# GestaltCogTeam/STEP

Hardware: AMD Instinct MI355X
Metric: training windows/sec on PEMS04, horizon-12 MAE parity, 1/2/4/8 MI355X (higher is better)
Workload: dtype f16 (TSFormer Q/K/weights) + bf16 (P, V, GraphWaveNet / graph-learner GEMMs) operands, f32 accumulate

## Files before the change

### include/step_hip.h

```cpp
#ifndef STEP_HIP_H
#define STEP_HIP_H

#include <stdint.h>

#ifdef __cplusplus
extern "C" {
#endif

const char* step_last_error(void);
int step_abi_version(void);

typedef struct StepGemm {
    int M, N, K, batch;
    const void* A; long sam, sak, sab; int a_bf16;
    const void* B; long sbk, sbn, sbb; int b_bf16;
    float* C; long ldc, scn, scb;
    float alpha;
    int accumulate;
    const float* bias; int relu;
    int splitk;
    int a_kblk; long a_kstride;
    int b_kblk; long b_kstride;
    int b_nblk; long b_nstride;
    int c_nblk; long c_nstride;
// ... 37 lines not shown
    float *bn3_w, *bn3_b, *bn3_rm, *bn3_rv;
    float *fc_out_w, *fc_out_b;
    float *fc_cat_w, *fc_cat_b;
    int gemm_bf16;
} StepDglParams;

long step_dgl_global_saved_floats(int N, int T);
long step_dgl_global_work_floats(int N, int T, int backward);
int step_dgl_global_forward(const float* series_nt, int N, int T, const StepDglParams* p, int training,
                            float momentum, float* saved, float* work, float* g, void* stream);
int step_dgl_global_backward(const float* series_nt, int N, int T, const StepDglParams* p, const float* saved,
                             const float* dg, float* work, const StepDglParams* grads, void* stream);
#define STEP_DGL_FRESH_FC_GRAD 16
int step_dgl_global_backward_phase(const float* series_nt, int N, int T, const StepDglParams* p, const float* saved,
                             const float* dg, float* work, const StepDglParams* grads, int phase, void* stream);

typedef struct StepDglShard { int own1; double count1, count2; } StepDglShard;
int step_dgl_global_forward_shard(const float* series_slice, int N, int Ts, const StepDglParams* p, int training, float momentum,
                                  float* saved, float* work, double* sums, float* g, const StepDglShard* shard, int phase,
                                  void* stream);
int step_dgl_global_backward_shard(const float* series_slice, int N, int Ts, const StepDglParams* p, const float* saved,
                                   const float* dg, float* work, const StepDglParams* grads, const StepDglShard* shard, int phase,
                                   void* stream);
long step_dgl_global_offset(int N, int T, int item);

long step_dgl_edges_saved_floats(int B, int N);
long step_dgl_edges_work_floats(int N);
long step_dgl_edges_theta_offset(int N);
int step_dgl_edges_forward(const float* g, int N, int B, const StepDglParams* p, const float* u, uint64_t seed,
                           float temperature, float* saved, float* theta_out, float* adj_out, void* stream);
int step_dgl_edges_backward(const float* g, int N, int B, const StepDglParams* p, const float* saved,
                            const float* dtheta, const float* dadj, float temperature, float* work,
                            const StepDglParams* grads, float* dg, void* aux_stream, void* stream);
int step_dgl_edges_backward_acc(const float* g, int N, int B, const StepDglParams* p, const float* saved,
                                const float* dtheta, const float* dadj, float temperature, float* work,
                                const StepDglParams* grads, float* dg, int dg_accumulate, void* aux_stream, void* stream);

typedef struct StepGwnetParams {
    float *nodevec1, *nodevec2;
    float *start_w, *start_b;
    float *filter_w[8], *filter_b[8];
    float *gate_w[8], *gate_b[8];
    float *skip_w[8], *skip_b[8];
    float *bn_w[8], *bn_b[8], *bn_rm[8], *bn_rv[8];
    float *gconv_w[8], *gconv_b[8];
    float *fc_his0_w, *fc_his0_b, *fc_his2_w, *fc_his2_b;
    float *end1_w, *end1_b, *end2_w, *end2_b;
    int gemm_bf16;
} StepGwnetParams;

long step_gwnet_saved_floats(int B, int N, int dropout);
long step_gwnet_work_floats(int B, int N, int backward);
long step_gwnet_saved_offset(int B, int N, int dropout, int item, int layer);
int step_gwnet_forward(const float* hist, int B, int N, int Cin, const float* hidden_last, const float* adj,
                       const StepGwnetParams* p, int training, float dropout_p, uint64_t seed, float momentum,
                       float* saved, float* work, float* pred, void* stream);
int step_gwnet_forward_phase(const float* hist, int B, int N, int Cin, const float* hidden_last, const float* adj,
                             const StepGwnetParams* p, int training, float dropout_p, uint64_t seed, float momentum,
                             float* saved, float* work, float* pred, int phase, void* stream);
int step_gwnet_backward(const float* hist, int B, int N, int Cin, const float* hidden_last, const StepGwnetParams* p,
                        const float* saved, float* work, const float* dpred, const StepGwnetParams* grads,
                        float* dadj, int dropout, void* aux_stream, void* leaf_stream, void* stream);

int step_pt_dropout(const float* x, float* y, long n, float p, uint64_t seed, uint32_t site, void* stream);
int step_pt_ffn_hidden_fwd(const float* x, const float* w1, const float* b1, long R, float p, uint64_t seed, uint32_t site,
                           uint16_t* hidden, void* stream);
int step_pt_ffn_hidden_bwd(const float* dy, const float* w2, const uint16_t* hidden, long R, float p, uint16_t* dhidden, void* stream);
int step_pt_colsum_bf16(const uint16_t* x, long rows, int cols, float* out, void* stream);
long step_pt_rows_linear_pack_bytes(int nkc, int nog);
int step_pt_rows_linear_pack(const float* w, long swo, long swi, int nkc, int nog, const float* bias, void* pack, void* stream);
int step_pt_rows_linear(const void* x, int x_bf16, long R, const void* pack, int nkc, int nog, void* y, int y_bf16, int accumulate, void* stream);
int step_pt_layer_pack(const float* wi, const float* bi, const float* wo, const float* bo, const float* w1, const float* b1, const float* w2,
                       const float* b2, void* ffn, void* qkv, void* o, void* da, void* dx, void* stream);
long step_pt_proj_wgrad_ws_floats(long R);
int step_pt_proj_wgrad(const float* x, const uint16_t* dqkv, const float* dov, const uint16_t* a, long R, float* ws, float* dwi, float* dbi, float* dwo,
                       void* stream);
int step_pt_ffn_fused_fwd_ln(const float* h1, long R, const void* pack, float p, const uint64_t* pool, long pool_words, uint64_t seed, uint32_t site_hidden,
                             uint32_t site_out, const float* gamma, const float* beta, float* pre, float* y, float* stats, void* stream);
int step_pt_rows_linear_ln(const uint16_t* x, long R, const void* pack, const float* res, float p, uint64_t seed, uint32_t site, const float* gamma,
                           const float* beta, float* pre, float* y, float* stats, void* stream);
int step_pt_embed_unmasked_fwd(const float* series, const int* um, const float* w, const float* b, const float* pos, long S, int L, int Pu, float p,
                               uint64_t seed, uint32_t site, float* x, void* stream);
int step_pt_embed_unmasked_bwd(const float* dx, const float* series, const int* um, long S, int L, int Pu, float p, uint64_t seed, uint32_t site,
                               float* dpos, float* dw, float* db, void* stream);
int step_pt_dec_input_bwd_sums(const float* dout, long S, int P, int Pu, float p, uint64_t seed, uint32_t site, const int* midx, float* dz, float* dpos,
                               float* dmask, void* stream);
long step_pt_ffn_pack_bytes(void);
long step_pt_ffn_wgrad_workgroups(long R);
long step_pt_ffn_wgrad_ws_floats(long R);
int step_pt_ffn_pack(const float* w1, const float* b1, const float* w2, const float* b2, void* pack, void* stream);
int step_pt_ffn_fused_fwd(const float* h1, long R, const void* pack, float p, const uint64_t* pool, long pool_words, uint64_t seed, uint32_t site,
                          float* f2, void* stream);
int step_pt_ffn_fused_bwd_data(const float* df2, const float* h1, long R, const void* pack, float p, const uint64_t* pool, long pool_words,
                               uint64_t seed, uint32_t site, float* dh1, void* stream);
int step_pt_ffn_fused_bwd_weights(const float* df2, const float* h1, long R, const void* pack, const float* b1, float p, const uint64_t* pool,
                                  long pool_words, uint64_t seed, uint32_t site, float* ws, float* dw1, float* db1, float* dw2, void* stream);
int step_pt_dropout_relu_mask(float* d, const float* relu_of, long n, float p, uint64_t seed, uint32_t site, void* stream);
int step_pt_add_dropout(const float* a, const float* b, float* out, long n, float p, uint64_t seed, uint32_t site, void* stream);
int step_pt_add_rows(float* x, long S, int P, const float* vec, const int* idx, void* stream);
int step_pt_sum_over_seq(const float* dx, long S, int ldp, int p_off, int p_cnt, const int* idx, float* dvec, void* stream);
int step_pt_token_gather(const float* src, long S, int P, const int* idx, int T, float scale, float* dst, void* stream);
int step_pt_token_scatter(const float* ddst, long S, int P, const int* idx, int T, float scale, float* dsrc, void* stream);
int step_pt_dec_input(const float* z, const float* mask_token, const float* pos, const int* midx, long S, int P, int Pu,
                      float p, uint64_t seed, uint32_t site, float* out, void* stream);
int step_pt_dec_input_bwd(const float* dout, long S, int P, int Pu, float p, uint64_t seed, uint32_t site, float* dz,
                          float* dm, void* stream);
// ... 103 lines not shown
```

### step_amd/csrc/gwnet.hip

```cpp
#include "common.h"
#include "step_internal.h"
#include <vector>

namespace {

constexpr int C = 32, CAT = 224, CS = 256, CE = 512, OUT = 12, NL = 8, HID = 96;
constexpr int TIN[NL] = {13, 12, 10, 9, 7, 6, 4, 3};
constexpr int DIL[NL] = {1, 2, 1, 2, 1, 2, 1, 2};
constexpr int TOUT[NL] = {12, 10, 9, 7, 6, 4, 3, 1};

__global__ void start_conv_kernel(const float* __restrict__ hist, int B, int N, int Cin, const float* __restrict__ w,
                                  const float* __restrict__ b, float* __restrict__ x0) {
    long idx = (long)blockIdx.x * 256 + threadIdx.x;
    long total = (long)B * N * 13 * C;
    if (idx >= total) return;
    int c = idx % C, t = (idx / C) % 13;
    long bn = idx / (C * 13);
    int n = bn % N, bb = bn / N;
    float v = b[c];
    if (t >= 1) {
        const float* src = hist + (((long)bb * 12 + (t - 1)) * N + n) * Cin;
        v += w[c * 2] * src[0] + w[c * 2 + 1] * src[1];
    }
    x0[idx] = v;
// ... 542 lines not shown
        long o[4];
        bool valid[4];
#pragma unroll
        for (int u = 0; u < 4; ++u) {
            const int j = j0 + 8 * u + jg;
            const int g = j / Tin, t = j - g * Tin;
            const long bnr = bn0 + g;
            valid[u] = j < njt && bnr < BN;
            const long bc = valid[u] ? bnr : 0;
            const int tc = valid[u] ? t : 0;
            o[u] = (bc * Tin + tc) * C + c;
            const bool tap1 = valid[u] && tc >= dil;
            dr[u] = (dres && tap1) ? dres[(bc * Tout + tc - dil) * C + c] : 0.f;
            yv[u] = yprev ? yprev[o[u]] : 0.f;
            float x = 0.f;
            if (valid[u] && tc < Tout) x += dxs[g * Tout + tc][c];
            if (tap1) x += dxs[g * Tout + tc - dil][32 + c];
            v[u] = x;
        }
#pragma unroll
        for (int u = 0; u < 4; ++u) {
            if (!valid[u]) continue;
            const float x = v[u] + dr[u];
            dx[o[u]] = x;
            s1 += x; s2 += x * (yv[u] - mean) * rstd;
        }
    }
    if (!yprev) return;
    red[jg][c] = s1; red[jg][32 + c] = s2;
    __syncthreads();
    if (threadIdx.x < 64) {
        float a = 0.f;
#pragma unroll
        for (int r = 0; r < 8; ++r) a += red[r][threadIdx.x];
        bsum[threadIdx.x] = a;
    }
    __syncthreads();
    add_block_sums(sums, bsum);
}

__global__ void im2col_kernel(XIn x, long BN, int Tin, int Tout, int dil, float* __restrict__ xcat) {
    long idx = (long)blockIdx.x * 256 + threadIdx.x;
    if (idx >= BN * Tout * 64) return;
    int k = idx % 64, t = (idx / 64) % Tout;
    long bn = idx / (64L * Tout);
    float v = x.src[(bn * Tin + t + (k >> 5) * dil) * C + (k & 31)];
    if (x.stat) v = v * x.stat[k & 31] + x.stat[32 + (k & 31)];
    xcat[idx] = v;
}
__global__ void unpack_skip_grad_kernel(const float* __restrict__ dwskip, SkipPtrs G) {
    const int o = blockIdx.x, k = threadIdx.x;
    G.w[k >> 5][o * C + (k & 31)] += dwskip[o * CS + k];
}
__global__ void head_combine_kernel(const float* __restrict__ skip, const float* __restrict__ h2, long n, float* __restrict__ xh) {
    long idx = (long)blockIdx.x * 256 + threadIdx.x;
    if (idx >= n) return;
    xh[idx] = fmaxf(skip[idx] + h2[idx], 0.f);
}
struct MPtr8 { float* p[8]; };
__global__ void add_to8_kernel(MPtr8 dst, const float* __restrict__ v, int n) {
    int i = blockIdx.x * 256 + threadIdx.x;
    if (i >= n) return;
    const float x = v[i];
#pragma unroll
    for (int k = 0; k < 8; ++k) dst.p[k][i] += x;
}
__global__ void relu_bwd_kernel(float* __restrict__ d, const float* __restrict__ y, long n) {
    long idx = (long)blockIdx.x * 256 + threadIdx.x;
    if (idx < n && !(y[idx] > 0.f)) d[idx] = 0.f;
}

__global__ __launch_bounds__(256) void rowsum_mod_kernel(const float* __restrict__ x, int cols, int mod, float* __restrict__ out) {
    __shared__ float red[4];
    const long row = blockIdx.x;
    float s = 0.f;
    for (int j = threadIdx.x; j < cols; j += 256) s += x[row * cols + j];
    s = wave_sum(s);
    if ((threadIdx.x & 63) == 0) red[threadIdx.x >> 6] = s;
    __syncthreads();
    if (threadIdx.x == 0) atomicAdd(&out[row % mod], red[0] + red[1] + red[2] + red[3]);
}

constexpr int ADJ_NSEG = 2 * (12 + 10 + 9 + 7 + 6 + 4 + 3);
struct AdjOffsets { long cat[NL - 1], dcat[NL - 1]; };
__global__ void adj_ktab_kernel(AdjOffsets o, int N, GemmKSeg* __restrict__ tab) {
    const int j = threadIdx.x, s = blockIdx.x;
    if (j >= ADJ_NSEG) return;
    constexpr int tout[NL - 1] = {12, 10, 9, 7, 6, 4, 3};
    int i = 0, rem = j >> 1;
    while (rem >= tout[i]) { rem -= tout[i]; ++i; }
    const int t = rem, pair = j & 1, T = tout[i];
    GemmKSeg g;
    g.a_off = o.cat[i] + (long)t * CAT + (pair == 0 ? (1 + 2 * s) * C : 0);
    g.b_off = o.dcat[i] + (long)t * CAT + (pair == 0 ? (2 + 2 * s) * C : (1 + 2 * s) * C);
    g.a_rs = g.b_rs = T * CAT;
    g.a_bs = g.b_bs = (long)N * T * CAT;
    tab[s * ADJ_NSEG + j] = g;
}

inline dim3 g1(long n) { return dim3((unsigned)((n + 255) / 256)); }

struct Carver {
    float* base;
    long used = 0;
    explicit Carver(float* b) : base(b) {}
    float* take(long n) {
        float* p = base ? base + used : nullptr;
        used += (n + 3) & ~3L;
        return p;
    }
// ... 109 lines not shown
        slots_to_bf16T_kernel<<<dim3(cdiv(N, 64), T, nsrc * B), 256, 0, st>>>(cat, src0, sstep, B, N, T, n8(N), xT);
        STEP_LAUNCH_CHECK("slots_to_bf16T");
        g.batch = 3 * B; g.batch0 = B;
        g.A = PT16; g.a_bf16 = 1; g.sam = n8(N); g.sak = 1; g.sab = (long)N * n8(N); g.sab1 = (long)B * N * n8(N);
        g.B = xT; g.b_bf16 = 1; g.sbk = 1; g.sbn = n8(N); g.sbb = (long)T * C * n8(N); g.sbb1 = nsrc == 1 ? 0 : (long)B * T * C * n8(N);
        g.scb = (long)N * T * CAT; g.scb1 = 2L * C;
        g.c_nblk = C; g.c_nstride = CAT;
        g.compute_bf16 = 1;
        return step_gemm_launch(g, st);
    }
    g.batch = 3 * B; g.batch0 = B;
    g.sab = (long)N * N; g.sab1 = (long)B * N * N;
    if (bf16) { g.A = PT16; g.a_bf16 = 1; g.sam = n8(N); g.sak = 1; g.sab = (long)N * n8(N); g.sab1 = (long)B * N * n8(N); }
    g.sbb = (long)N * T * CAT; g.sbb1 = (long)sstep * C;
    g.scb = (long)N * T * CAT; g.scb1 = 2L * C;
    g.b_nblk = C; g.b_nstride = CAT; g.c_nblk = C; g.c_nstride = CAT;
    g.compute_bf16 = bf16;
    return step_gemm_launch(g, st);
}
int nconv_bwd_data3(const float* PTstk, const uint16_t* P16, float* dcat, int src0, int dst0, int dstep, int B, int N, int T, int bf16,
                    uint16_t* xT, hipStream_t st) {
    StepGemm g = gemm_desc(N, T * C, N, PTstk, 1, N, dcat + src0 * C, (long)T * CAT, 1, dcat + dst0 * C, (long)T * CAT);
    if (bf16 && xT) {
        slots_to_bf16T_kernel<<<dim3(cdiv(N, 64), T, 3 * B), 256, 0, st>>>(dcat, src0, 2, B, N, T, n8(N), xT);
        STEP_LAUNCH_CHECK("slots_to_bf16T");
        g.batch = 3 * B; g.batch0 = B;
        g.A = P16; g.a_bf16 = 1; g.sam = n8(N); g.sak = 1; g.sab = (long)N * n8(N); g.sab1 = (long)B * N * n8(N);
        g.B = xT; g.b_bf16 = 1; g.sbk = 1; g.sbn = n8(N); g.sbb = (long)T * C * n8(N); g.sbb1 = (long)B * T * C * n8(N);
        g.scb = (long)N * T * CAT; g.scb1 = (long)dstep * C;
        g.c_nblk = C; g.c_nstride = CAT;
        g.accumulate = dstep == 0 ? 2 : 1;
        g.compute_bf16 = 1;
        return step_gemm_launch(g, st);
    }
    g.batch = 3 * B; g.batch0 = B;
    g.sab = (long)N * N; g.sab1 = (long)B * N * N;
    if (bf16) { g.A = P16; g.a_bf16 = 1; g.sam = n8(N); g.sak = 1; g.sab = (long)N * n8(N); g.sab1 = (long)B * N * n8(N); }
    g.sbb = (long)N * T * CAT; g.sbb1 = 2L * C;
    g.scb = (long)N * T * CAT; g.scb1 = (long)dstep * C;
    g.b_nblk = C; g.b_nstride = CAT; g.c_nblk = C; g.c_nstride = CAT;
    g.accumulate = dstep == 0 ? 2 : 1;
    g.compute_bf16 = bf16;
    return step_gemm_launch(g, st);
}
}

extern "C" long step_gwnet_saved_floats(int B, int N, int dropout) { return carve_saved(nullptr, B, N, dropout != 0).total; }
extern "C" long step_gwnet_work_floats(int B, int N, int backward) { return carve_work(nullptr, B, N, backward != 0).total; }
extern "C" long step_gwnet_saved_offset(int B, int N, int dropout, int item, int layer) {
    Saved s = carve_saved((float*)16, B, N, dropout != 0);
    float* p = item == 0 ? s.mask[layer] : item == 1 ? s.y[layer] : s.bnstat[layer];
    return p ? (long)(p - (float*)16) : -1;
}

template <bool BF16>
static int gwnet_layers_forward(const StepGwnetParams* p, const Saved& S, const Work& W, int B, int N, bool training, float drop_p,
                                uint64_t seed, float momentum, bool dead_bn7, const StepDynState* dyn, hipStream_t st,
                                bool first_tcn_only = false, bool skip_first_tcn = false) {
    const long BN = (long)B * N;
    for (int i = 0; i < (first_tcn_only ? 1 : NL); ++i) {
        const int Tin = TIN[i], Tout = TOUT[i], dil = DIL[i];
        const long npos = BN * Tout;
        BnFwd bn = {nullptr, nullptr, nullptr, nullptr, training ? 1 : 0, momentum, nullptr, (double)BN * Tin, nullptr};
        if (i > 0) {
            bn.gamma = p->bn_w[i - 1]; bn.beta = p->bn_b[i - 1]; bn.rm = p->bn_rm[i - 1]; bn.rv = p->bn_rv[i - 1];
            bn.stat = S.bnstat[i - 1]; bn.sums = W.acc64 + (long)(i - 1) * NCOPY * 64;
        }
        if (!(i == 0 && skip_first_tcn)) {
            tcn_fwd_kernel<BF16><<<(unsigned)cdiv(npos, 128), 256, 0, st>>>(i == 0 ? S.x0 : S.y[i - 1], bn, npos, Tin, Tout, dil, W.wcat + i * 4096,
                                                                            W.bcat + i * 64, S.tf[i], S.sg[i], S.cat[i], S.zlast, i);
            STEP_LAUNCH_CHECK("tcn_fwd");
        }
        if (first_tcn_only) break;
        if (i == NL - 1 && !(dead_bn7 && training)) break;
        STEP_TRY(nconv_fwd3(S.Pstk, S.PT16, S.cat[i], 0, 0, 1, B, N, Tout, BF16, W.xT, st));
        STEP_TRY(nconv_fwd3(S.Pstk, S.PT16, S.cat[i], 1, 2, 2, B, N, Tout, BF16, W.xT, st));
        const XIn xin = {i == 0 ? S.x0 : S.y[i - 1], i == 0 ? nullptr : S.bnstat[i - 1]};
        const bool dead = i == NL - 1;
        mix_fwd_kernel<BF16><<<(unsigned)cdiv(npos, 64), 256, 0, st>>>(S.cat[i], p->gconv_w[i], p->gconv_b[i], xin, npos, Tin, Tout, dil, drop_p,
                                                                       (uint32_t)seed, (uint32_t)(seed >> 32), (uint32_t)i, dead ? W.m7 : S.mask[i],
                                                                       dead ? W.y7 : S.y[i], W.acc64 + (long)i * NCOPY * 64, dyn);
        STEP_LAUNCH_CHECK("mix_fwd");
        if (dead) {
            const BnFwd b7 = {p->bn_w[i], p->bn_b[i], p->bn_rm[i], p->bn_rv[i], 1, momentum, S.bnstat[i], (double)npos, W.acc64 + (long)i * NCOPY * 64};
            bn_stats_only_kernel<<<1, 64, 0, st>>>(b7);
            STEP_LAUNCH_CHECK("bn7_stats");
        }
    }
    return STEP_OK;
}

static int pack_weights(const StepGwnetParams* p, const Work& W, hipStream_t st) {
    GatePtrs gp;
    SkipPtrs sp;
    MixPtrs mp;
    for (int i = 0; i < NL; ++i) {
        gp.wf[i] = p->filter_w[i]; gp.bf[i] = p->filter_b[i]; gp.wg[i] = p->gate_w[i]; gp.bg[i] = p->gate_b[i];
        sp.w[i] = p->skip_w[i]; sp.b[i] = p->skip_b[i];
        if (i < NL - 1) mp.w[i] = p->gconv_w[i];
    }
    pack_weights_kernel<<<384 + 7 * 28, 256, 0, st>>>(gp, sp, mp, W.wcat, W.wcatT, W.bcat, W.wskip, W.bsum, W.wmixT);
    STEP_LAUNCH_CHECK("pack_weights");
    return STEP_OK;
}

extern "C" int step_gwnet_forward(const float* hist, int B, int N, int Cin, const float* hidden_last, const float* adj,
// ... 24 lines not shown
    const bool use_drop = train && dropout_p > 0.f;
    Saved S = carve_saved(saved, B, N, use_drop);
    Work W = carve_work(work, B, N, false);
    const long BN = (long)B * N;
    const int allbf16 = p->gemm_bf16;

    const long NN = (long)N * N;
    const bool dead_bn7 = (training & 2) != 0;
    if (do_prep) {
        STEP_TRY(zero((float*)W.acc64, 2L * NL * NCOPY * 64, st));
        start_conv_kernel<<<g1(BN * 13 * C), 256, 0, st>>>(hist, B, N, Cin, p->start_w, p->start_b, S.x0);
        STEP_LAUNCH_CHECK("start_conv");
        {
            StepGemm g = gemm_desc(N, N, 10, p->nodevec1, 10, 1, p->nodevec2, N, 1, S.Madp, N);
            STEP_TRY(step_gemm_launch(g, st));
            softmax_relu_rows_kernel<<<N, 256, 0, st>>>(S.Madp, N, S.Pa);
            replicate_adp_kernel<<<g1(NN), 256, 0, st>>>(S.Pa, N, B, S.Pstk + 2 * B * NN, S.PTstk + 2 * B * NN);
            STEP_LAUNCH_CHECK("adp_softmax");
        }
        STEP_TRY(pack_weights(p, W, st));
        if (allbf16) STEP_TRY(gwnet_layers_forward<true>(p, S, W, B, N, train, use_drop ? dropout_p : 0.f, seed, momentum, dead_bn7, dyn, st, true, false));
        else STEP_TRY(gwnet_layers_forward<false>(p, S, W, B, N, train, use_drop ? dropout_p : 0.f, seed, momentum, dead_bn7, dyn, st, true, false));
    }
    if (do_layers) {
        row_sums_kernel<<<(unsigned)BN, 256, 0, st>>>(adj, N, S.rs, S.cs);
        {
            int slices = cdiv(512, cdiv(N, 64) * B);
            if (slices > cdiv(N, 64)) slices = cdiv(N, 64);
            if (slices < 1) slices = 1;
            col_sums_kernel<<<dim3(cdiv(N, 64), slices, B), 256, 0, st>>>(adj, N, S.cs);
        }
        rw_build_kernel<<<dim3(cdiv(N, 32), cdiv(N, 32), B), 256, 0, st>>>(adj, N, S.rs, S.cs, S.Pstk, S.Pstk + B * NN, S.PTstk,
                                                                           S.PTstk + B * NN);
        STEP_LAUNCH_CHECK("rw_build");
        if (p->gemm_bf16) {
            const long rows = 3L * B * N;
            stacks_to_bf16_kernel<<<dim3((unsigned)cdiv(rows * (n8(N) / 2), 256), 2), 256, 0, st>>>(S.Pstk, S.PTstk, rows, N, n8(N), S.P16,
                                                                                                   S.PT16);
            STEP_LAUNCH_CHECK("stacks_to_bf16");
        }
        if (allbf16) STEP_TRY(gwnet_layers_forward<true>(p, S, W, B, N, train, use_drop ? dropout_p : 0.f, seed, momentum, dead_bn7, dyn, st, false, true));
        else STEP_TRY(gwnet_layers_forward<false>(p, S, W, B, N, train, use_drop ? dropout_p : 0.f, seed, momentum, dead_bn7, dyn, st, false, true));
    }

    if (do_his) {
        StepGemm g = gemm_desc((int)BN, CE, HID, hidden_last, HID, 1, p->fc_his0_w, 1, HID, S.h1, CE);
        g.bias = p->fc_his0_b; g.relu = 1;
        g.compute_bf16 = allbf16; STEP_TRY(step_gemm_launch(g, st));
        StepGemm g2 = gemm_desc((int)BN, CS, CE, S.h1, CE, 1, p->fc_his2_w, 1, CE, S.h2, CS);
        g2.bias = p->fc_his2_b; g2.relu = 1;
        g2.compute_bf16 = allbf16; STEP_TRY(step_gemm_launch(g2, st));
    }
    if (do_head) {
        StepGemm gs = gemm_desc((int)BN, CS, CS, S.zlast, CS, 1, W.wskip, 1, CS, S.skip, CS);
        gs.bias = W.bsum;
        gs.compute_bf16 = allbf16; STEP_TRY(step_gemm_launch(gs, st));
        head_combine_kernel<<<g1(BN * CS), 256, 0, st>>>(S.skip, S.h2, BN * CS, S.xh);
        STEP_LAUNCH_CHECK("head_combine");
        StepGemm g3 = gemm_desc((int)BN, CE, CS, S.xh, CS, 1, p->end1_w, 1, CS, S.e1, CE);
        g3.bias = p->end1_b; g3.relu = 1;
        g3.compute_bf16 = allbf16; STEP_TRY(step_gemm_launch(g3, st));
        StepGemm g4 = gemm_desc(N, OUT, CE, S.e1, CE, 1, p->end2_w, 1, CE, pred, 1);
        g4.batch = B; g4.sab = (long)N * CE; g4.scb = (long)OUT * N; g4.scn = N;
        g4.bias = p->end2_b;
        g4.compute_bf16 = allbf16; STEP_TRY(step_gemm_launch(g4, st));
    }
    return STEP_OK;
}

template <bool BF16>
static int gwnet_layers_backward(const StepGwnetParams* p, const StepGwnetParams* grads, const Saved& S, const Work& W, int B, int N,
                                 float** dx0, hipStream_t st, AuxLane& lane, AuxLane& leaves, hipEvent_t* adj_done) {
    const long BN = (long)B * N;
    float* dx_next = nullptr;
    float* dxbuf[2] = {W.dxa, W.dxb};
    {
        AdjOffsets o;
        for (int i = 0; i < NL - 1; ++i) { o.cat[i] = S.cat[i] - S.cat[0]; o.dcat[i] = W.dcat[i] - W.dcat[0]; }
        adj_ktab_kernel<<<3, 128, 0, st>>>(o, N, W.ktab);
        STEP_LAUNCH_CHECK("adj_ktab");
    }
    static const bool adj_pieces = []() { const char* e = getenv("STEP_ADJ_PIECES"); return !(e && e[0] == '0'); }();
    bool adj_first = true;
    auto adj_piece = [&](int lo, int hi, hipStream_t on_stream) -> int {
        int seg0 = 0, nseg = 0;
        for (int i = 0; i < lo; ++i) seg0 += 2 * TOUT[i];
        for (int i = lo; i <= hi; ++i) nseg += 2 * TOUT[i];
        StepGemm g = gemm_desc(N, N, 32 * nseg, S.cat[0], 0, 1, W.dcat[0], 1, 0, W.dPstk, N);
        g.batch = 3 * B; g.batch0 = B;
        g.scb = (long)N * N; g.scb1 = (long)B * N * N;
        g.compute_bf16 = BF16;
        g.accumulate = adj_first ? 0 : 1;
        adj_first = false;
        return step_gemm_segmented_launch(g, W.ktab + seg0, ADJ_NSEG, on_stream);
    };
    for (int i = NL - 1; i >= 0; --i) {
        const int Tin = TIN[i], Tout = TOUT[i], dil = DIL[i];
        const long npos = BN * Tout;
        const float* cat = S.cat[i];
        if (i < NL - 1) {
            const BnBwd bn = {p->bn_w[i], S.bnstat[i], grads->bn_w[i], grads->bn_b[i], (double)npos, W.acc64 + (long)i * NCOPY * 64};
            mix_bwd_kernel<BF16><<<(unsigned)cdiv(npos, 128), 256, 0, st>>>(dx_next, S.y[i], bn, S.mask[i], W.wmixT + i * (C * CAT), npos, W.dres, W.dh[i],
                                                                            W.dcat[i]);
            STEP_LAUNCH_CHECK("mix_bwd");
            STEP_TRY(nconv_bwd_data3(S.PTstk, S.P16, W.dcat[i], 2, 1, 2, B, N, Tout, BF16, W.xT, st));
            STEP_TRY(nconv_bwd_data3(S.PTstk, S.P16, W.dcat[i], 1, 0, 0, B, N, Tout, BF16, W.xT, st));
            if (adj_pieces && i == 0) { STEP_TRY(adj_piece(0, 0, lane.fork())); *adj_done = lane.done(); }
        }
        float* dx = dxbuf[i & 1];
        tcn_bwd_kernel<BF16><<<(unsigned)cdiv(BN, TB_ROWS / Tout), 256, 0, st>>>(i < NL - 1 ? W.dcat[i] : nullptr, W.dskip, i, S.tf[i], S.sg[i],
                                                                                W.wcatT + i * 4096, i < NL - 1 ? W.dres : nullptr, BN, Tin, Tout, dil,
                                                                                W.dpre[i], dx, i > 0 ? S.y[i - 1] : nullptr,
                                                                                i > 0 ? S.bnstat[i - 1] : nullptr,
                                                                                i > 0 ? W.acc64 + (long)(i - 1) * NCOPY * 64 : nullptr);
        STEP_LAUNCH_CHECK("tcn_bwd");
        const XIn xin = {i == 0 ? S.x0 : S.y[i - 1], i == 0 ? nullptr : S.bnstat[i - 1]};
        hipEvent_t ev = leaves.on ? leaves.mark() : lane.mark();
        if (adj_pieces && i == 4) STEP_TRY(adj_piece(4, 6, lane.after(ev)));
        if (adj_pieces && i == 2) STEP_TRY(adj_piece(2, 3, lane.after(ev)));
        if (adj_pieces && i == 1) STEP_TRY(adj_piece(1, 1, lane.after(ev)));
        hipStream_t leaf = leaves.after(ev);
        if (i < NL - 1) {
            StepGemm gw = gemm_desc(C, CAT, (int)npos, W.dh[i], 1, C, cat, CAT, 1, grads->gconv_w[i], CAT);
            gw.accumulate = 2; gw.splitk = -1;
            gw.a_rowsum = grads->gconv_b[i];
            gw.compute_bf16 = BF16; STEP_TRY(step_gemm_launch(gw, leaf));
        }
        im2col_kernel<<<g1(npos * 64), 256, 0, leaf>>>(xin, BN, Tin, Tout, dil, W.xcat[i]);
        STEP_LAUNCH_CHECK("im2col");
        StepGemm gw = gemm_desc(64, 64, (int)npos, W.dpre[i], 1, 64, W.xcat[i], 64, 1, W.dwcat + i * 4096, 64);
        gw.accumulate = 2; gw.splitk = -1;
        gw.a_rowsum = W.dbcat + i * 64;
        gw.compute_bf16 = BF16; STEP_TRY(step_gemm_launch(gw, leaf));
        dx_next = dx;
    }
    *dx0 = dx_next;
    if (!adj_pieces) STEP_TRY(adj_piece(0, NL - 2, lane.fork()));
    return STEP_OK;
}

extern "C" int step_gwnet_backward(const float* hist, int B, int N, int Cin, const float* hidden_last, const StepGwnetParams* p,
                                   const float* saved, float* work, const float* dpred, const StepGwnetParams* grads,
                                   float* dadj, int dropout, void* aux_stream, void* leaf_stream, void* stream) {
    STEP_REQUIRE(hist && hidden_last && p && saved && work && dpred && grads && dadj, "gwnet_backward: null argument");
    STEP_REQUIRE(B > 0 && N > 0 && Cin >= 2, "gwnet_backward: bad sizes");
    hipStream_t st = (hipStream_t)stream;
    AuxLane lane(st, (hipStream_t)aux_stream);
    AuxLane leaves(st, leaf_stream ? (hipStream_t)leaf_stream : (hipStream_t)aux_stream, 64);
    Saved S = carve_saved((float*)saved, B, N, dropout != 0);
    Work W = carve_work(work, B, N, true);
    const long BN = (long)B * N;
    const int allbf16 = p->gemm_bf16;
    auto split_for = [](long) { return -1; };

    STEP_TRY(pack_weights(p, W, st));
    STEP_TRY(zero(W.dwcat, (long)((float*)W.acc64 - W.dwcat) + 2L * NL * NCOPY * 64, st));
    const long NN = (long)N * N;

    {
        StepGemm g = gemm_desc(N, CE, OUT, dpred, 1, N, p->end2_w, CE, 1, W.d_e1, CE);
        g.batch = B; g.sab = (long)OUT * N; g.scb = (long)N * CE;
        STEP_TRY(step_gemm_launch(g, st));
        relu_bwd_kernel<<<g1(BN * CE), 256, 0, st>>>(W.d_e1, S.e1, BN * CE);
        StepGemm gx = gemm_desc((int)BN, CS, CE, W.d_e1, CE, 1, p->end1_w, CS, 1, W.d_xh, CS);
        gx.compute_bf16 = allbf16; STEP_TRY(step_gemm_launch(gx, st));
        relu_bwd_kernel<<<g1(BN * CS), 256, 0, st>>>(W.d_xh, S.xh, BN * CS);
        {
            hipStream_t leaf = leaves.fork();
            StepGemm gz = gemm_desc((int)BN, CS, CS, W.d_xh, CS, 1, W.wskip, CS, 1, W.dskip, CS);
            gz.compute_bf16 = allbf16; STEP_TRY(step_gemm_launch(gz, st));
            {
                StepGemm gw = gemm_desc(OUT, CE, N, dpred, N, 1, S.e1, CE, 1, grads->end2_w, CE);
                gw.batch = B; gw.sab = (long)OUT * N; gw.sbb = (long)N * CE; gw.scb = 0; gw.accumulate = 2;
                STEP_TRY(step_gemm_launch(gw, leaf));
                rowsum_mod_kernel<<<B * OUT, 256, 0, leaf>>>(dpred, N, OUT, grads->end2_b);
                STEP_LAUNCH_CHECK("end2_bias_grad");
                StepGemm gw1 = gemm_desc(CE, CS, (int)BN, W.d_e1, 1, CE, S.xh, CS, 1, grads->end1_w, CS);
                gw1.accumulate = 2; gw1.splitk = split_for(BN);
                gw1.a_rowsum = grads->end1_b;
                gw1.compute_bf16 = allbf16; STEP_TRY(step_gemm_launch(gw1, leaf));
            }
            STEP_TRY(zero(W.bsum, CS, leaf));
            STEP_TRY(step_colsum_launch(W.d_xh, BN, CS, CS, W.bsum, leaf));
            MPtr8 gb;
            for (int i = 0; i < NL; ++i) gb.p[i] = grads->skip_b[i];
            add_to8_kernel<<<1, 256, 0, leaf>>>(gb, W.bsum, CS);
            StepGemm gws = gemm_desc(CS, CS, (int)BN, W.d_xh, 1, CS, S.zlast, CS, 1, W.dwskip, CS);
            gws.accumulate = 2; gws.splitk = split_for(BN);
            gws.compute_bf16 = allbf16; STEP_TRY(step_gemm_launch(gws, leaf));
            if (hipMemcpyAsync(W.d_h2, W.d_xh, (size_t)BN * CS * sizeof(float), hipMemcpyDeviceToDevice, leaf) != hipSuccess) {
                step_set_error("gwnet_backward: copy failed");
                return STEP_ERR_HIP;
            }
            relu_bwd_kernel<<<g1(BN * CS), 256, 0, leaf>>>(W.d_h2, S.h2, BN * CS);
            StepGemm gw2 = gemm_desc(CS, CE, (int)BN, W.d_h2, 1, CS, S.h1, CE, 1, grads->fc_his2_w, CE);
            gw2.accumulate = 2; gw2.splitk = split_for(BN);
            gw2.a_rowsum = grads->fc_his2_b;
            gw2.compute_bf16 = allbf16; STEP_TRY(step_gemm_launch(gw2, leaf));
            StepGemm gh1 = gemm_desc((int)BN, CE, CS, W.d_h2, CS, 1, p->fc_his2_w, CE, 1, W.d_h1, CE);
            gh1.compute_bf16 = allbf16; STEP_TRY(step_gemm_launch(gh1, leaf));
            relu_bwd_kernel<<<g1(BN * CE), 256, 0, leaf>>>(W.d_h1, S.h1, BN * CE);
            StepGemm gw0 = gemm_desc(CE, HID, (int)BN, W.d_h1, 1, CE, hidden_last, HID, 1, grads->fc_his0_w, HID);
            gw0.accumulate = 2; gw0.splitk = split_for(BN);
            gw0.a_rowsum = grads->fc_his0_b;
            gw0.compute_bf16 = allbf16; STEP_TRY(step_gemm_launch(gw0, leaf));
        }
    }

    float* dx0 = nullptr;
    hipEvent_t adj_done = nullptr;
    if (allbf16) STEP_TRY(gwnet_layers_backward<true>(p, grads, S, W, B, N, &dx0, st, lane, leaves, &adj_done));
    else STEP_TRY(gwnet_layers_backward<false>(p, grads, S, W, B, N, &dx0, st, lane, leaves, &adj_done));
    STEP_TRY(lane.wait_done(adj_done));
    static const bool tail_leaves = []() { const char* e = getenv("STEP_TAIL_LEAVES"); return !(e && e[0] == '0'); }();
    if (!tail_leaves) STEP_TRY(leaves.join());
    hipStream_t leaf = tail_leaves ? leaves.fork() : st;
    row_dot_kernel<<<(unsigned)BN, 256, 0, st>>>(W.dPstk, S.Pstk, N, W.rf);
    row_dot_kernel<<<(unsigned)BN, 256, 0, st>>>(W.dPstk + B * NN, S.Pstk + B * NN, N, W.rb);
    rw_bwd_kernel<<<dim3(cdiv(N, 32), cdiv(N, 32), B), 256, 0, st>>>(W.dPstk, W.dPstk + B * NN, N, S.rs, S.cs, W.rf, W.rb, dadj);
    STEP_LAUNCH_CHECK("rw_bwd");
    {
        GatePtrs gg;
        SkipPtrs sg;
// ... 26 lines not shown
```

Measured before the change: 2397.

## Fuse GraphWaveNet output head GEMM chain into single forward and backward kernels

Replaces the forward head sequence (skip GEMM, combine/relu, end1 GEMM, end2 GEMM) with one MFMA kernel per 32-row tile. Intermediates stay in LDS, and xh/e1 are still written out for the backward pass. The backward head (end2 transpose GEMM, relu mask, end1 GEMM, relu mask, skip GEMM) is fused the same way. This removes several launches and round-trips of large intermediates through global memory. In exchange it adds a large hand-tuned kernel with heavy LDS use and fixed per-tile weight reloads, which may underutilize the GPU compared with the tuned general GEMM.

```diff
diff --git a/include/step_hip.h b/include/step_hip.h
--- a/include/step_hip.h
+++ b/include/step_hip.h
@@ -113,6 +113,7 @@
 long step_gwnet_saved_floats(int B, int N, int dropout);
 long step_gwnet_work_floats(int B, int N, int backward);
 long step_gwnet_saved_offset(int B, int N, int dropout, int item, int layer);
+extern const int step_gwnet_head_rows;
 int step_gwnet_forward(const float* hist, int B, int N, int Cin, const float* hidden_last, const float* adj,
                        const StepGwnetParams* p, int training, float dropout_p, uint64_t seed, float momentum,
                        float* saved, float* work, float* pred, void* stream);
diff --git a/step_amd/csrc/gwnet.hip b/step_amd/csrc/gwnet.hip
--- a/step_amd/csrc/gwnet.hip
+++ b/step_amd/csrc/gwnet.hip
@@ -618,10 +618,290 @@
     const int o = blockIdx.x, k = threadIdx.x;
     G.w[k >> 5][o * C + (k & 31)] += dwskip[o * CS + k];
 }
-__global__ void head_combine_kernel(const float* __restrict__ skip, const float* __restrict__ h2, long n, float* __restrict__ xh) {
-    long idx = (long)blockIdx.x * 256 + threadIdx.x;
-    if (idx >= n) return;
-    xh[idx] = fmaxf(skip[idx] + h2[idx], 0.f);
+#ifndef STEP_HEAD_ROWS
+#define STEP_HEAD_ROWS 32
+#endif
+constexpr int HEAD_ROWS = STEP_HEAD_ROWS, HEAD_WAVES = 8, HEAD_THREADS = 64 * HEAD_WAVES;
+constexpr int XLD = CS + 4, ELD = CE + 4;
+constexpr int HEAD_LDS_BYTES = HEAD_ROWS * (XLD + ELD) * (int)sizeof(float);
+static_assert(HEAD_THREADS == CE && HEAD_ROWS * OUT <= HEAD_THREADS && HEAD_WAVES * HEAD_ROWS * OUT <= HEAD_ROWS * XLD, "head kernels: thread / LDS layout");
+
+template <int H> struct HeadTile;
+template <> struct HeadTile<32> {
+    typedef f32x16 Acc;
+    static constexpr int KS = 16, NE = 16;
+    static __device__ __forceinline__ int idx(int lane) { return lane & 31; }
+    static __device__ __forceinline__ int part(int lane) { return lane >> 5; }
+    static __device__ __forceinline__ int row(int e, int part) { return (e & 3) + 8 * (e >> 2) + 4 * part; }
+    static __device__ __forceinline__ int koff(int part, int j) { return 4 * part + (j & 3) + 8 * (j >> 2); }
+    static __device__ __forceinline__ void load(const float* chunk, int part, float* v) { load8h(chunk, part, v); }
+    template <bool BF16> static __device__ __forceinline__ void mma(Acc& acc, const float* a, const float* b) { mma16<BF16>(acc, a, b); }
+};
+template <> struct HeadTile<16> {
+    typedef f32x4 Acc;
+    static constexpr int KS = 32, NE = 4;
+    static __device__ __forceinline__ int idx(int lane) { return lane & 15; }
+    static __device__ __forceinline__ int part(int lane) { return lane >> 4; }
+    static __device__ __forceinline__ int row(int e, int part) { return 4 * part + e; }
+    static __device__ __forceinline__ int koff(int part, int j) { return 4 * part + (j & 3) + 16 * (j >> 2); }
+    static __device__ __forceinline__ void load(const float* chunk, int part, float* v) { load8q(chunk, part, v); }
+    template <bool BF16> static __device__ __forceinline__ void mma(Acc& acc, const float* a, const float* b) { mma32_16<BF16>(acc, a, b); }
+};
+
+template <bool BF16, int H, int TPW, int K, int KCK, bool KCONTIG>
+__device__ __forceinline__ void head_product(typename HeadTile<H>::Acc (&acc)[TPW], const float* as, int lda, const float* __restrict__ w,
+                                             int ldw, int col0, int k0, int ix, int bix, int part) {
+    typedef HeadTile<H> T;
+    constexpr int KC = KCK / T::KS, NCH = K / KCK;
+    static_assert(K % KCK == 0 && KCK % T::KS == 0, "head_product: chunking");
+    float b[2][TPW][KC][8];
+    auto loadb = [&](int buf, int ch) {
+#pragma unroll
+        for (int t = 0; t < TPW; ++t)
+#pragma unroll
+            for (int s = 0; s < KC; ++s) {
+                const int col = col0 + t * H + bix, k = k0 + (ch * KC + s) * T::KS;
+                if constexpr (KCONTIG) {
+                    T::load(w + (long)col * ldw + k, part, b[buf][t][s]);
+                } else {
+#pragma unroll
+                    for (int j = 0; j < 8; ++j) b[buf][t][s][j] = w[(long)(k + T::koff(part, j)) * ldw + col];
+                }
+            }
+    };
+    loadb(0, 0);
+#pragma unroll
+    for (int ch = 0; ch < NCH; ++ch) {
+        if (ch + 1 < NCH) loadb((ch + 1) & 1, ch + 1);
+        __builtin_amdgcn_sched_barrier(0);
+#pragma unroll
+        for (int s = 0; s < KC; ++s) {
+            float a[8];
+            T::load(as + ix * lda + k0 + (ch * KC + s) * T::KS, part, a);
+#pragma unroll
+            for (int t = 0; t < TPW; ++t) T::template mma<BF16>(acc[t], a, b[ch & 1][t][s]);
+        }
+        __builtin_amdgcn_sched_barrier(0);
+    }
+}
+
+template <bool BF16, int H>
+__global__ __launch_bounds__(HEAD_THREADS) void head_fwd_kernel(const float* __restrict__ zlast, const float* __restrict__ h2,
+                                                                const float* __restrict__ wskip, const float* __restrict__ bsum,
+                                                                const float* __restrict__ w1, const float* __restrict__ b1,
+                                                                const float* __restrict__ w2, const float* __restrict__ b2, long BN, int N,
+                                                                float* __restrict__ xh, float* __restrict__ e1, float* __restrict__ pred) {
+    typedef HeadTile<H> T;
+    extern __shared__ __align__(16) float head_lds[];
+    float* xs = head_lds;
+    float* es = head_lds + H * XLD;
+    const int tid = threadIdx.x, lane = tid & 63, wave = tid >> 6, ix = T::idx(lane), part = T::part(lane);
+    const long r0 = (long)blockIdx.x * H;
+    const int nrow = BN - r0 < H ? (int)(BN - r0) : H;
+    static_assert(H * (CS / 4) % HEAD_THREADS == 0, "head_fwd: zlast tile load");
+#pragma unroll
+    for (int it = 0; it < H * (CS / 4) / HEAD_THREADS; ++it) {
+        const int i = it * HEAD_THREADS + tid;
+        const int r = i / (CS / 4), c4 = i % (CS / 4);
+        const long gr = r0 + (r < nrow ? r : nrow - 1);
+        *(float4*)(es + r * XLD + 4 * c4) = *(const float4*)(zlast + gr * CS + 4 * c4);
+    }
+    {
+        constexpr int TPW = CS / H / HEAD_WAVES;
+        const int col0 = wave * TPW * H;
+        float hv[TPW][T::NE], bv[TPW];
+#pragma unroll
+        for (int t = 0; t < TPW; ++t) {
+            bv[t] = bsum[col0 + t * H + ix];
+#pragma unroll
+            for (int e = 0; e < T::NE; ++e) {
+                const int r = T::row(e, part);
+                hv[t][e] = h2[(r0 + (r < nrow ? r : nrow - 1)) * CS + col0 + t * H + ix];
+            }
+        }
+        typename T::Acc acc[TPW];
+#pragma unroll
+        for (int t = 0; t < TPW; ++t)
+#pragma unroll
+            for (int e = 0; e < T::NE; ++e) acc[t][e] = 0.f;
+        __syncthreads();
+        head_product<BF16, H, TPW, CS, 64, true>(acc, es, XLD, wskip, CS, col0, 0, ix, ix, part);
+#pragma unroll
+        for (int t = 0; t < TPW; ++t)
+#pragma unroll
+            for (int e = 0; e < T::NE; ++e) {
+                const int r = T::row(e, part), c = col0 + t * H + ix;
+                const float v = fmaxf(acc[t][e] + bv[t] + hv[t][e], 0.f);
+                xs[r * XLD + c] = v;
+                if (r < nrow) xh[(r0 + r) * CS + c] = v;
+            }
+    }
+    __syncthreads();
+    {
+        constexpr int TPW = CE / H / HEAD_WAVES;
+        const int col0 = wave * TPW * H;
+        float bv[TPW];
+#pragma unroll
+        for (int t = 0; t < TPW; ++t) bv[t] = b1[col0 + t * H + ix];
+        typename T::Acc acc[TPW];
+#pragma unroll
+        for (int t = 0; t < TPW; ++t)
+#pragma unroll
+            for (int e = 0; e < T::NE; ++e) acc[t][e] = 0.f;
+        head_product<BF16, H, TPW, CS, 64, true>(acc, xs, XLD, w1, CS, col0, 0, ix, ix, part);
+#pragma unroll
+        for (int t = 0; t < TPW; ++t)
+#pragma unroll
+            for (int e = 0; e < T::NE; ++e) {
+                const int r = T::row(e, part), c = col0 + t * H + ix;
+                const float v = fmaxf(acc[t][e] + bv[t], 0.f);
+                es[r * ELD + c] = v;
+                if (r < nrow) e1[(r0 + r) * CE + c] = v;
+            }
+    }
+    __syncthreads();
+    {
+        constexpr int KW = CE / HEAD_WAVES;
+        typename T::Acc acc[1];
+#pragma unroll
+        for (int e = 0; e < T::NE; ++e) acc[0][e] = 0.f;
+        const bool real = ix < OUT;
+        head_product<BF16, H, 1, KW, KW, true>(acc, es, ELD, w2, CE, 0, wave * KW, ix, real ? ix : 0, part);
+        if (real) {
+#pragma unroll
+            for (int e = 0; e < T::NE; ++e) xs[(wave * H + T::row(e, part)) * OUT + ix] = acc[0][e];
+        }
+    }
+    __syncthreads();
+    if (tid < H * OUT) {
+        const int o = tid / H, r = tid % H;
+        float part8[HEAD_WAVES];
+#pragma unroll
+        for (int w = 0; w < HEAD_WAVES; ++w) part8[w] = xs[(w * H + r) * OUT + o];
+#pragma unroll
+        for (int s = 1; s < HEAD_WAVES; s *= 2)
+#pragma unroll
+            for (int w = 0; w < HEAD_WAVES; w += 2 * s) part8[w] += part8[w + s];
+        const float v = part8[0];
+        if (r < nrow) {
+            const long gr = r0 + r, b = gr / N;
+            pred[(b * OUT + o) * N + (gr - b * N)] = v + b2[o];
+        }
+    }
+}
+
+template <bool BF16, int H>
+__global__ __launch_bounds__(HEAD_THREADS) void head_bwd_kernel(const float* __restrict__ dpred, const float* __restrict__ w2,
+                                                                const float* __restrict__ e1, const float* __restrict__ w1,
+                                                                const float* __restrict__ xh, const float* __restrict__ wskip, long BN, int N,
+                                                                float* __restrict__ d_e1, float* __restrict__ d_xh, float* __restrict__ dskip) {
+    typedef HeadTile<H> T;
+    extern __shared__ __align__(16) float head_lds[];
+    float* dxs = head_lds;
+    float* des = head_lds + H * XLD;
+    const int tid = threadIdx.x, lane = tid & 63, wave = tid >> 6, ix = T::idx(lane), part = T::part(lane);
+    const long r0 = (long)blockIdx.x * H;
+    const int nrow = BN - r0 < H ? (int)(BN - r0) : H;
+    float* dp = dxs;
+    if (tid < H * OUT) {
+        const int o = tid / H, r = tid % H;
+        const long gr = r0 + (r < nrow ? r : nrow - 1), b = gr / N;
+        dp[r * OUT + o] = dpred[(b * OUT + o) * N + (gr - b * N)];
+    }
+    {
+        const int li = lane & 31, lk = lane >> 5;
+        float a[2][4], b[2][2][4], ev[2][16];
+#pragma unroll
+        for (int t = 0; t < 2; ++t) {
+            const int col = (2 * wave + t) * 32 + li;
+#pragma unroll
+            for (int q = 0; q < 2; ++q)
+#pragma unroll
+                for (int j = 0; j < 4; ++j) {
+                    const int k = 8 * q + 4 * lk + j;
+                    b[t][q][j] = k < OUT ? w2[k * CE + col] : 0.f;
+                }
+#pragma unroll
+            for (int e = 0; e < 16; ++e) {
+                const int r = (e & 3) + 8 * (e >> 2) + 4 * lk;
+                ev[t][e] = r < H ? e1[(r0 + (r < nrow ? r : nrow - 1)) * CE + col] : 0.f;
+            }
+        }
+        __syncthreads();
+#pragma unroll
+        for (int q = 0; q < 2; ++q)
+#pragma unroll
+            for (int j = 0; j < 4; ++j) {
+                const int k = 8 * q + 4 * lk + j;
+                a[q][j] = (li < H && k < OUT) ? dp[li * OUT + k] : 0.f;
+            }
+#pragma unroll
+        for (int t = 0; t < 2; ++t) {
+            f32x16 acc, acc2;
+#pragma unroll
+            for (int e = 0; e < 16; ++e) { acc[e] = 0.f; acc2[e] = 0.f; }
+#pragma unroll
+            for (int q = 0; q < 2; ++q)
+#pragma unroll
+                for (int j = 0; j < 4; j += 2) {
+                    acc = __builtin_amdgcn_mfma_f32_32x32x2f32(a[q][j], b[t][q][j], acc, 0, 0, 0);
+                    acc2 = __builtin_amdgcn_mfma_f32_32x32x2f32(a[q][j + 1], b[t][q][j + 1], acc2, 0, 0, 0);
+                }
+            const int col = (2 * wave + t) * 32 + li;
+#pragma unroll
+            for (int e = 0; e < 16; ++e) {
+                const int r = (e & 3) + 8 * (e >> 2) + 4 * lk;
+                if (r >= H) continue;
+                const float v = (r < nrow && ev[t][e] > 0.f) ? acc[e] + acc2[e] : 0.f;
+                des[r * ELD + col] = v;
+                if (r < nrow) d_e1[(r0 + r) * CE + col] = v;
+            }
+        }
+    }
+    __syncthreads();
+    constexpr int TPW = CS / H / HEAD_WAVES;
+    const int col0 = wave * TPW * H;
+    {
+        float xv[TPW][T::NE];
+#pragma unroll
+        for (int t = 0; t < TPW; ++t)
+#pragma unroll
+            for (int e = 0; e < T::NE; ++e) {
+                const int r = T::row(e, part);
+                xv[t][e] = xh[(r0 + (r < nrow ? r : nrow - 1)) * CS + col0 + t * H + ix];
+            }
+        typename T::Acc acc[TPW];
+#pragma unroll
+        for (int t = 0; t < TPW; ++t)
+#pragma unroll
+            for (int e = 0; e < T::NE; ++e) acc[t][e] = 0.f;
+        head_product<BF16, H, TPW, CE, 64, false>(acc, des, ELD, w1, CS, col0, 0, ix, ix, part);
+#pragma unroll
+        for (int t = 0; t < TPW; ++t)
+#pragma unroll
+            for (int e = 0; e < T::NE; ++e) {
+                const int r = T::row(e, part), c = col0 + t * H + ix;
+                const float v = (r < nrow && xv[t][e] > 0.f) ? acc[t][e] : 0.f;
+                dxs[r * XLD + c] = v;
+                if (r < nrow) d_xh[(r0 + r) * CS + c] = v;
+            }
+    }
+    __syncthreads();
+    {
+        typename T::Acc acc[TPW];
+#pragma unroll
+        for (int t = 0; t < TPW; ++t)
+#pragma unroll
+            for (int e = 0; e < T::NE; ++e) acc[t][e] = 0.f;
+        head_product<BF16, H, TPW, CS, 64, false>(acc, dxs, XLD, wskip, CS, col0, 0, ix, ix, part);
+#pragma unroll
+        for (int t = 0; t < TPW; ++t)
+#pragma unroll
+            for (int e = 0; e < T::NE; ++e) {
+                const int r = T::row(e, part);
+                if (r < nrow) dskip[(r0 + r) * CS + col0 + t * H + ix] = acc[t][e];
+            }
+    }
 }
 struct MPtr8 { float* p[8]; };
 __global__ void add_to8_kernel(MPtr8 dst, const float* __restrict__ v, int n) {
@@ -837,6 +1117,7 @@
     float* p = item == 0 ? s.mask[layer] : item == 1 ? s.y[layer] : s.bnstat[layer];
     return p ? (long)(p - (float*)16) : -1;
 }
+extern "C" const int step_gwnet_head_rows = HEAD_ROWS;
 
 template <bool BF16>
 static int gwnet_layers_forward(const StepGwnetParams* p, const Saved& S, const Work& W, int B, int N, bool training, float drop_p,
@@ -967,18 +1248,17 @@
         g2.compute_bf16 = allbf16; STEP_TRY(step_gemm_launch(g2, st));
     }
     if (do_head) {
-        StepGemm gs = gemm_desc((int)BN, CS, CS, S.zlast, CS, 1, W.wskip, 1, CS, S.skip, CS);
-        gs.bias = W.bsum;
-        gs.compute_bf16 = allbf16; STEP_TRY(step_gemm_launch(gs, st));
-        head_combine_kernel<<<g1(BN * CS), 256, 0, st>>>(S.skip, S.h2, BN * CS, S.xh);
-        STEP_LAUNCH_CHECK("head_combine");
-        StepGemm g3 = gemm_desc((int)BN, CE, CS, S.xh, CS, 1, p->end1_w, 1, CS, S.e1, CE);
-        g3.bias = p->end1_b; g3.relu = 1;
-        g3.compute_bf16 = allbf16; STEP_TRY(step_gemm_launch(g3, st));
-        StepGemm g4 = gemm_desc(N, OUT, CE, S.e1, CE, 1, p->end2_w, 1, CE, pred, 1);
-        g4.batch = B; g4.sab = (long)N * CE; g4.scb = (long)OUT * N; g4.scn = N;
-        g4.bias = p->end2_b;
-        g4.compute_bf16 = allbf16; STEP_TRY(step_gemm_launch(g4, st));
+        const unsigned nblk = (unsigned)cdiv(BN, HEAD_ROWS);
+        if (allbf16) {
+            STEP_TRY(step_raise_lds_once((const void*)head_fwd_kernel<true, HEAD_ROWS>, HEAD_LDS_BYTES, "gwnet_forward"));
+            head_fwd_kernel<true, HEAD_ROWS><<<nblk, HEAD_THREADS, HEAD_LDS_BYTES, st>>>(S.zlast, S.h2, W.wskip, W.bsum, p->end1_w, p->end1_b, p->end2_w,
+                                                                                         p->end2_b, BN, N, S.xh, S.e1, pred);
+        } else {
+            STEP_TRY(step_raise_lds_once((const void*)head_fwd_kernel<false, HEAD_ROWS>, HEAD_LDS_BYTES, "gwnet_forward"));
+            head_fwd_kernel<false, HEAD_ROWS><<<nblk, HEAD_THREADS, HEAD_LDS_BYTES, st>>>(S.zlast, S.h2, W.wskip, W.bsum, p->end1_w, p->end1_b, p->end2_w,
+                                                                                          p->end2_b, BN, N, S.xh, S.e1, pred);
+        }
+        STEP_LAUNCH_CHECK("head_fwd");
     }
     return STEP_OK;
 }
@@ -1073,17 +1353,19 @@
     const long NN = (long)N * N;
 
     {
-        StepGemm g = gemm_desc(N, CE, OUT, dpred, 1, N, p->end2_w, CE, 1, W.d_e1, CE);
-        g.batch = B; g.sab = (long)OUT * N; g.scb = (long)N * CE;
-        STEP_TRY(step_gemm_launch(g, st));
-        relu_bwd_kernel<<<g1(BN * CE), 256, 0, st>>>(W.d_e1, S.e1, BN * CE);
-        StepGemm gx = gemm_desc((int)BN, CS, CE, W.d_e1, CE, 1, p->end1_w, CS, 1, W.d_xh, CS);
-        gx.compute_bf16 = allbf16; STEP_TRY(step_gemm_launch(gx, st));
-        relu_bwd_kernel<<<g1(BN * CS), 256, 0, st>>>(W.d_xh, S.xh, BN * CS);
+        const unsigned nblk = (unsigned)cdiv(BN, HEAD_ROWS);
+        if (allbf16) {
+            STEP_TRY(step_raise_lds_once((const void*)head_bwd_kernel<true, HEAD_ROWS>, HEAD_LDS_BYTES, "gwnet_backward"));
+            head_bwd_kernel<true, HEAD_ROWS><<<nblk, HEAD_THREADS, HEAD_LDS_BYTES, st>>>(dpred, p->end2_w, S.e1, p->end1_w, S.xh, W.wskip, BN, N, W.d_e1,
+                                                                                         W.d_xh, W.dskip);
+        } else {
+            STEP_TRY(step_raise_lds_once((const void*)head_bwd_kernel<false, HEAD_ROWS>, HEAD_LDS_BYTES, "gwnet_backward"));
+            head_bwd_kernel<false, HEAD_ROWS><<<nblk, HEAD_THREADS, HEAD_LDS_BYTES, st>>>(dpred, p->end2_w, S.e1, p->end1_w, S.xh, W.wskip, BN, N, W.d_e1,
+                                                                                          W.d_xh, W.dskip);
+        }
+        STEP_LAUNCH_CHECK("head_bwd");
         {
             hipStream_t leaf = leaves.fork();
-            StepGemm gz = gemm_desc((int)BN, CS, CS, W.d_xh, CS, 1, W.wskip, CS, 1, W.dskip, CS);
-            gz.compute_bf16 = allbf16; STEP_TRY(step_gemm_launch(gz, st));
             {
                 StepGemm gw = gemm_desc(OUT, CE, N, dpred, N, 1, S.e1, CE, 1, grads->end2_w, CE);
                 gw.batch = B; gw.sab = (long)OUT * N; gw.sbb = (long)N * CE; gw.scb = 0; gw.accumulate = 2;
```

After: 2414, median of 6. No clear change (+0.7%).
